# Ascend-Research/HeadPoseEstimation-WHENet

Hardware: NVIDIA H100
Metric: head-crops/sec @224x224 bf16 (higher is better)
Workload: dtype bf16

## Files before the change

headposeestimation-whenet_b200/csrc/kernels_simt.cuh:

```cuda
#pragma once
#include <cuda_bf16.h>
#include <cuda_fp16.h>
#include <cuda_runtime.h>
#include <stdint.h>

namespace whenet {

template <typename T> struct Store;
template <> struct Store<float> {
    static constexpr int VEC = 4;
    __device__ static __forceinline__ float ld(const float* p) { return *p; }
    __device__ static __forceinline__ void st(float* p, float v) { *p = v; }
    __device__ static __forceinline__ float rnd(float v) { return v; }
};
template <> struct Store<__nv_bfloat16> {
    static constexpr int VEC = 8;
    __device__ static __forceinline__ float ld(const __nv_bfloat16* p) { return __bfloat162float(*p); }
    __device__ static __forceinline__ void st(__nv_bfloat16* p, float v) { *p = __float2bfloat16_rn(v); }
    __device__ static __forceinline__ float rnd(float v) { return __bfloat162float(__float2bfloat16_rn(v)); }
};
template <> struct Store<__half> {
    static constexpr int VEC = 8;
    __device__ static __forceinline__ float ld(const __half* p) { return __half2float(*p); }
    __device__ static __forceinline__ void st(__half* p, float v) { *p = __float2half_rn(v); }
    __device__ static __forceinline__ float rnd(float v) { return __half2float(__float2half_rn(v)); }
};

__device__ __forceinline__ void ld4(const float* p, float (&v)[4]) {
    float4 t = *reinterpret_cast<const float4*>(p);
    v[0] = t.x; v[1] = t.y; v[2] = t.z; v[3] = t.w;
}
__device__ __forceinline__ void ld4(const __nv_bfloat16* p, float (&v)[4]) {
    uint2 t = *reinterpret_cast<const uint2*>(p);
    __nv_bfloat162 a = *reinterpret_cast<__nv_bfloat162*>(&t.x), b = *reinterpret_cast<__nv_bfloat162*>(&t.y);
    float2 fa = __bfloat1622float2(a), fb = __bfloat1622float2(b);
    v[0] = fa.x; v[1] = fa.y; v[2] = fb.x; v[3] = fb.y;
}
__device__ __forceinline__ void ld4(const __half* p, float (&v)[4]) {
    uint2 t = *reinterpret_cast<const uint2*>(p);
    __half2 a = *reinterpret_cast<__half2*>(&t.x), b = *reinterpret_cast<__half2*>(&t.y);
    float2 fa = __half22float2(a), fb = __half22float2(b);
    v[0] = fa.x; v[1] = fa.y; v[2] = fb.x; v[3] = fb.y;
}
__device__ __forceinline__ void st4(float* p, const float (&v)[4]) {
    *reinterpret_cast<float4*>(p) = make_float4(v[0], v[1], v[2], v[3]);
}
__device__ __forceinline__ void st4(__nv_bfloat16* p, const float (&v)[4]) {
    __nv_bfloat162 a = __floats2bfloat162_rn(v[0], v[1]), b = __floats2bfloat162_rn(v[2], v[3]);
    uint2 t; t.x = *reinterpret_cast<uint32_t*>(&a); t.y = *reinterpret_cast<uint32_t*>(&b);
    *reinterpret_cast<uint2*>(p) = t;
}
__device__ __forceinline__ void st4(__half* p, const float (&v)[4]) {
    __half2 a = __floats2half2_rn(v[0], v[1]), b = __floats2half2_rn(v[2], v[3]);
    uint2 t; t.x = *reinterpret_cast<uint32_t*>(&a); t.y = *reinterpret_cast<uint32_t*>(&b);
    *reinterpret_cast<uint2*>(p) = t;
}

template <typename T> __device__ __forceinline__ void ld8(const T* p, float (&v)[8]) {
    float a[4], b[4];
    ld4(p, a); ld4(p + 4, b);
#pragma unroll
    for (int i = 0; i < 4; ++i) { v[i] = a[i]; v[4 + i] = b[i]; }
}
template <> __device__ __forceinline__ void ld8<__nv_bfloat16>(const __nv_bfloat16* p, float (&v)[8]) {
    uint4 t = *reinterpret_cast<const uint4*>(p);
    const __nv_bfloat162* h = reinterpret_cast<const __nv_bfloat162*>(&t);
#pragma unroll
    for (int i = 0; i < 4; ++i) { float2 f = __bfloat1622float2(h[i]); v[2 * i] = f.x; v[2 * i + 1] = f.y; }
}
template <> __device__ __forceinline__ void ld8<__half>(const __half* p, float (&v)[8]) {
    uint4 t = *reinterpret_cast<const uint4*>(p);
    const __half2* h = reinterpret_cast<const __half2*>(&t);
#pragma unroll
    for (int i = 0; i < 4; ++i) { float2 f = __half22float2(h[i]); v[2 * i] = f.x; v[2 * i + 1] = f.y; }
}
template <typename T> __device__ __forceinline__ void st8(T* p, const float (&v)[8]) {
    float a[4] = {v[0], v[1], v[2], v[3]}, b[4] = {v[4], v[5], v[6], v[7]};
    st4(p, a); st4(p + 4, b);
}
template <> __device__ __forceinline__ void st8<__nv_bfloat16>(__nv_bfloat16* p, const float (&v)[8]) {
    uint4 t; __nv_bfloat162* h = reinterpret_cast<__nv_bfloat162*>(&t);
#pragma unroll
    for (int i = 0; i < 4; ++i) h[i] = __floats2bfloat162_rn(v[2 * i], v[2 * i + 1]);
    *reinterpret_cast<uint4*>(p) = t;
}
template <> __device__ __forceinline__ void st8<__half>(__half* p, const float (&v)[8]) {
    uint4 t; __half2* h = reinterpret_cast<__half2*>(&t);
#pragma unroll
    for (int i = 0; i < 4; ++i) h[i] = __floats2half2_rn(v[2 * i], v[2 * i + 1]);
    *reinterpret_cast<uint4*>(p) = t;
}

__device__ __forceinline__ float swish_f(float x) { return x / (1.0f + expf(-x)); }
__device__ __forceinline__ float sigmoid_f(float x) { return 1.0f / (1.0f + expf(-x)); }
__device__ __forceinline__ float swish_fast(float x) {
    const float h = 0.5f * x;
    float t;
    asm("tanh.approx.f32 %0, %1;" : "=f"(t) : "f"(h));
    return fmaf(h, t, h);
}

__device__ __forceinline__ float swish_from_half(float h) {
    float t;
    asm("tanh.approx.f32 %0, %1;" : "=f"(t) : "f"(h));
    return fmaf(h, t, h);
}

template <typename T, bool IN_U8>
__global__ void __launch_bounds__(256) stem_kernel(const void* __restrict__ in_, T* __restrict__ out,
                                                   const float* __restrict__ w,
                                                   const float* __restrict__ bias,
                                                   const float* __restrict__ lut,
                                                   int n_img) {
    __shared__ float s_w[27 * 32];
    __shared__ float s_lut[3 * 256];
    for (int i = threadIdx.x; i < 27 * 32; i += 256) s_w[i] = w[i];
    if (IN_U8)
        for (int i = threadIdx.x; i < 768; i += 256) s_lut[i] = lut[i];
    __syncthreads();
    const long long total = (long long)n_img * 112 * 112 * 4;
    long long gid = (long long)blockIdx.x * 256 + threadIdx.x;
    if (gid >= total) return;
    const int cg = (int)(gid & 3);
    long long pix = gid >> 2;
    const int ox = (int)(pix % 112); pix /= 112;
    const int oy = (int)(pix % 112);
    const int n = (int)(pix / 112);
    float acc[8];
#pragma unroll
    for (int i = 0; i < 8; ++i) acc[i] = bias[cg * 8 + i];
#pragma unroll
    for (int ky = 0; ky < 3; ++ky) {
        const int iy = 2 * oy + ky;
        if (iy >= 224) continue;
#pragma unroll
        for (int kx = 0; kx < 3; ++kx) {
            const int ix = 2 * ox + kx;
            if (ix >= 224) continue;
            const long long base = (((long long)n * 224 + iy) * 224 + ix) * 3;
#pragma unroll
            for (int ci = 0; ci < 3; ++ci) {
                float x;
                if (IN_U8) x = s_lut[ci * 256 + reinterpret_cast<const uint8_t*>(in_)[base + ci]];
                else x = reinterpret_cast<const float*>(in_)[base + ci];
                const float* wr = &s_w[((ky * 3 + kx) * 3 + ci) * 32 + cg * 8];
#pragma unroll
                for (int i = 0; i < 8; ++i) acc[i] = fmaf(x, wr[i], acc[i]);
            }
        }
    }
#pragma unroll
    for (int i = 0; i < 8; ++i) acc[i] = swish_f(acc[i]);
    st8(out + (gid >> 2) * 32 + cg * 8, acc);
}

struct StemParams { float w[27 * 32]; float b[32]; };

template <typename T, bool IN_U8, bool FAST>
__global__ void __launch_bounds__(224) stem_tile_kernel(const void* __restrict__ in_, T* __restrict__ out,
                                                        const __grid_constant__ StemParams sp,
                                                        const float* __restrict__ lut) {
    constexpr int ROWF = 225 * 3 + 1;
    __shared__ float s_in[5 * ROWF];
    __shared__ float s_lut[768];
    const int tid = threadIdx.x;
    const int n = blockIdx.y, oy0 = blockIdx.x * 2;
    if (IN_U8) {
        for (int i = tid; i < 768; i += 224) s_lut[i] = lut[i];
        __syncthreads();
    }
    if (IN_U8) {
        const uint8_t* src = reinterpret_cast<const uint8_t*>(in_) + (long long)n * 224 * 224 * 3;
        for (int v = tid; v < 5 * 42; v += 224) {
            const int r = v / 42, q = v - r * 42;
            const int iy = 2 * oy0 + r;
            float* dst = &s_in[r * ROWF + q * 16];
            if (iy < 224) {
                const uint4 raw = *reinterpret_cast<const uint4*>(src + (long long)iy * 672 + q * 16);
                const uint8_t* b = reinterpret_cast<const uint8_t*>(&raw);
#pragma unroll
                for (int j = 0; j < 16; ++j) dst[j] = s_lut[((q * 16 + j) % 3) * 256 + b[j]];
            } else {
#pragma unroll
                for (int j = 0; j < 16; ++j) dst[j] = 0.f;
            }
        }
    } else {
        const float* src = reinterpret_cast<const float*>(in_) + (long long)n * 224 * 224 * 3;
        for (int v = tid; v < 5 * 168; v += 224) {
            const int r = v / 168, q = v - r * 168;
            const int iy = 2 * oy0 + r;
            float4 x = make_float4(0.f, 0.f, 0.f, 0.f);
            if (iy < 224) x = *reinterpret_cast<const float4*>(src + (long long)iy * 672 + q * 4);
            float* dst = &s_in[r * ROWF + q * 4];
            dst[0] = x.x; dst[1] = x.y; dst[2] = x.z; dst[3] = x.w;
        }
    }
    if (tid < 15) s_in[(tid / 3) * ROWF + 672 + tid % 3] = 0.f;
    __syncthreads();
    const int oyl = tid / 112, ox = tid - oyl * 112;
    float2 acc2[16];
#pragma unroll
    for (int c = 0; c < 16; ++c) acc2[c] = make_float2(sp.b[2 * c], sp.b[2 * c + 1]);
#pragma unroll
    for (int ky = 0; ky < 3; ++ky) {
        const float* row = &s_in[(2 * oyl + ky) * ROWF + 6 * ox];
#pragma unroll
        for (int t = 0; t < 9; ++t) {
            const float x = row[t];
            const float2 xx = make_float2(x, x);
#pragma unroll
            for (int c = 0; c < 16; ++c) {
                const float2 w2 = make_float2(sp.w[(ky * 9 + t) * 32 + 2 * c], sp.w[(ky * 9 + t) * 32 + 2 * c + 1]);
                acc2[c].x = fmaf(xx.x, w2.x, acc2[c].x);
                acc2[c].y = fmaf(xx.y, w2.y, acc2[c].y);
            }
        }
    }
    float acc[32];
#pragma unroll
    for (int c = 0; c < 16; ++c) { acc[2 * c] = acc2[c].x; acc[2 * c + 1] = acc2[c].y; }
    T* dst = out + (((long long)n * 112 + oy0 + oyl) * 112 + ox) * 32;
#pragma unroll
    for (int g = 0; g < 4; ++g) {
        float o[8];
#pragma unroll
        for (int j = 0; j < 8; ++j) o[j] = FAST ? swish_fast(acc[g * 8 + j]) : swish_f(acc[g * 8 + j]);
        st8<T>(dst + g * 8, o);
    }
}

template <typename T, bool SWISH, bool GATE, bool RESID>
__global__ void __launch_bounds__(256) pw_conv_kernel(const T* __restrict__ A, const float* __restrict__ W,
                                                      const float* __restrict__ bias, const float* __restrict__ gate,
                                                      const T* __restrict__ resid, T* __restrict__ out,
                                                      long long M, int K, int N, int hw) {
    constexpr int BM = 64, BN = 64, BK = 16;
    __shared__ float As[BK][BM + 4];
    __shared__ float Bs[BK][BN];
    const int tid = threadIdx.x;
    const int tx = tid & 15, ty = tid >> 4;
    const long long m0 = (long long)blockIdx.x * BM;
    const int n0 = blockIdx.y * BN;
    float acc[4][4];
#pragma unroll
    for (int i = 0; i < 4; ++i)
#pragma unroll
        for (int j = 0; j < 4; ++j) acc[i][j] = 0.f;

    const int a_row = tid >> 2, a_k = (tid & 3) * 4;
    const int b_k = tid >> 4, b_n = (tid & 15) * 4;
    const long long a_m = m0 + a_row;
    const bool a_ok = a_m < M;
    const float* gate_row = GATE ? gate + (a_ok ? (a_m / hw) : 0) * K : nullptr;

    for (int k0 = 0; k0 < K; k0 += BK) {
        float av[4] = {0.f, 0.f, 0.f, 0.f};
        if (a_ok && k0 + a_k < K) {
            ld4(A + a_m * K + k0 + a_k, av);
            if (GATE) {
                float g[4]; ld4(gate_row + k0 + a_k, g);
#pragma unroll
                for (int i = 0; i < 4; ++i) av[i] *= g[i];
            }
        }
#pragma unroll
        for (int i = 0; i < 4; ++i) As[a_k + i][a_row] = av[i];
        float4 bv = make_float4(0.f, 0.f, 0.f, 0.f);
        if (k0 + b_k < K && n0 + b_n < N) bv = *reinterpret_cast<const float4*>(W + (long long)(k0 + b_k) * N + n0 + b_n);
        *reinterpret_cast<float4*>(&Bs[b_k][b_n]) = bv;
        __syncthreads();
#pragma unroll
        for (int k = 0; k < BK; ++k) {
            float4 a4 = *reinterpret_cast<const float4*>(&As[k][ty * 4]);
            float4 b4 = *reinterpret_cast<const float4*>(&Bs[k][tx * 4]);
            const float a[4] = {a4.x, a4.y, a4.z, a4.w}, b[4] = {b4.x, b4.y, b4.z, b4.w};
#pragma unroll
            for (int i = 0; i < 4; ++i)
#pragma unroll
                for (int j = 0; j < 4; ++j) acc[i][j] = fmaf(a[i], b[j], acc[i][j]);
        }
        __syncthreads();
    }
    const int n = n0 + tx * 4;
    if (n >= N) return;
    float bb[4]; ld4(bias + n, bb);
#pragma unroll
    for (int i = 0; i < 4; ++i) {
        const long long m = m0 + ty * 4 + i;
        if (m >= M) break;
        float v[4];
#pragma unroll
        for (int j = 0; j < 4; ++j) {
            float x = acc[i][j] + bb[j];
            v[j] = SWISH ? swish_f(x) : x;
        }
        if (RESID) {
            float r[4]; ld4(resid + m * N + n, r);
#pragma unroll
            for (int j = 0; j < 4; ++j) v[j] += r[j];
        }
        st4(out + m * N + n, v);
    }
}

template <typename T, int KS, int S>
__global__ void __launch_bounds__(256) dw_conv_kernel(const T* __restrict__ in, const float* __restrict__ w,
                                                      const float* __restrict__ bias, T* __restrict__ out,
                                                      float* __restrict__ partial,
                                                      int Hin, int Ho, int C, int pad, int rows) {
    extern __shared__ float s_red[];
    const int cv = threadIdx.x, py = threadIdx.y, PY = blockDim.y;
    const int c0 = cv * 8;
    const int n = blockIdx.y, tile = blockIdx.x;
    const int r0 = tile * rows;
    const int r1 = min(Ho, r0 + rows);
    const int npix = (r1 - r0) * Ho;
    const T* in_n = in + (long long)n * Hin * Hin * C;
    T* out_n = out + (long long)n * Ho * Ho * C;
    float bb[8];
#pragma unroll
    for (int i = 0; i < 8; ++i) bb[i] = bias[c0 + i];
    float sum[8];
#pragma unroll
    for (int i = 0; i < 8; ++i) sum[i] = 0.f;
    for (int p = py; p < npix; p += PY) {
        const int oy = r0 + p / Ho, ox = p % Ho;
        float acc[8];
#pragma unroll
        for (int i = 0; i < 8; ++i) acc[i] = bb[i];
#pragma unroll
        for (int ky = 0; ky < KS; ++ky) {
            const int iy = oy * S + ky - pad;
            if (iy < 0 || iy >= Hin) continue;
#pragma unroll
            for (int kx = 0; kx < KS; ++kx) {
                const int ix = ox * S + kx - pad;
                if (ix < 0 || ix >= Hin) continue;
                float x[8], ww[8];
                ld8(in_n + ((long long)iy * Hin + ix) * C + c0, x);
                ld8(w + (ky * KS + kx) * C + c0, ww);
#pragma unroll
                for (int i = 0; i < 8; ++i) acc[i] = fmaf(x[i], ww[i], acc[i]);
            }
        }
#pragma unroll
        for (int i = 0; i < 8; ++i) { acc[i] = swish_f(acc[i]); }
        st8(out_n + ((long long)oy * Ho + ox) * C + c0, acc);
#pragma unroll
        for (int i = 0; i < 8; ++i) sum[i] += Store<T>::rnd(acc[i]);
    }
#pragma unroll
    for (int i = 0; i < 8; ++i) s_red[py * C + c0 + i] = sum[i];
    __syncthreads();
    if (py == 0) {
        float tot[8];
#pragma unroll
        for (int i = 0; i < 8; ++i) tot[i] = 0.f;
        for (int y = 0; y < PY; ++y)
#pragma unroll
            for (int i = 0; i < 8; ++i) tot[i] += s_red[y * C + c0 + i];
        float* dst = partial + ((long long)n * gridDim.x + tile) * C + c0;
#pragma unroll
        for (int i = 0; i < 8; ++i) dst[i] = tot[i];
    }
}


template <typename T, int KS, int S, int R, bool FAST>
__global__ void __launch_bounds__(256) dw_strip_kernel(const T* __restrict__ in, const float* __restrict__ w,
                                                       const float* __restrict__ bias, T* __restrict__ out,
                                                       float* __restrict__ partial,
                                                       int Hin, int Ho, int C, int pad, int rows) {
    extern __shared__ float s_red[];
    constexpr int NCOL = (R - 1) * S + KS;
    const int cv = threadIdx.x, py = threadIdx.y, PY = blockDim.y;
    const int c0 = cv * 8;
    const int n = blockIdx.y, tile = blockIdx.x;
    const int r0 = tile * rows;
    const int r1 = min(Ho, r0 + rows);
    const int spr = (Ho + R - 1) / R;
    const int nstrips = (r1 - r0) * spr;
// ... 409 lines not shown
```

headposeestimation-whenet_b200/csrc/whenet_api.cu:

```cuda
#include <cuda_bf16.h>
#include <cuda_fp16.h>
#include <cuda_runtime.h>

#include <algorithm>
#include <atomic>
#include <cmath>
#include <cstdarg>
#include <cstdio>
#include <cstdlib>
#include <cstring>
#include <map>
#include <string>
#include <thread>
#include <type_traits>
#include <vector>

#include "../../include/whenet_b200.h"
#include "api_error.h"
#include "kernels_simt.cuh"
#include "kernels_tc.cuh"
#include "kernels_fused.cuh"
#include "kernels_crop.cuh"
#include "kernels_overlay.cuh"
#include "kernels_k2.cuh"
// ... 356 lines not shown
int make_tmap_kd_e(CUtensorMap* tm, const void* base, int n, int H, int C, int cc, int pw) {
    auto fn = tmap_encode_fn();
    if (!fn) return fail(WHENET_ECUDA, "cuTensorMapEncodeTiled is not available from this driver");
    const cuuint64_t dims[4] = {(cuuint64_t)C, (cuuint64_t)H, (cuuint64_t)H, (cuuint64_t)n};
    const cuuint64_t strides[3] = {(cuuint64_t)C * 2, (cuuint64_t)H * C * 2, (cuuint64_t)H * H * C * 2};
    const cuuint32_t box[4] = {(cuuint32_t)cc, (cuuint32_t)pw, (cuuint32_t)pw, 1};
    const cuuint32_t estr[4] = {1, 1, 1, 1};
    const CUresult r = fn(tm, CU_TENSOR_MAP_DATA_TYPE_FLOAT16, 4, const_cast<void*>(base), dims, strides, box, estr, CU_TENSOR_MAP_INTERLEAVE_NONE,
                          CU_TENSOR_MAP_SWIZZLE_NONE, CU_TENSOR_MAP_L2_PROMOTION_L2_128B, CU_TENSOR_MAP_FLOAT_OOB_FILL_NONE);
    if (r != CUDA_SUCCESS) return fail(WHENET_ECUDA, "cuTensorMapEncodeTiled(KD tile %dx%dx%dx%d, box %dx%dx%d) failed: %d", n, H, H, C, pw, pw, cc, (int)r);
    return 0;
}
int make_tmap_k1x_in(CUtensorMap* tm, const void* base, int n, int H, int C, int iw, int row_bytes) {
    auto fn = tmap_encode_fn();
    if (!fn) return fail(WHENET_ECUDA, "cuTensorMapEncodeTiled is not available from this driver");
    const cuuint64_t dims[4] = {(cuuint64_t)C, (cuuint64_t)H, (cuuint64_t)H, (cuuint64_t)n};
    const cuuint64_t strides[3] = {(cuuint64_t)C * 2, (cuuint64_t)H * C * 2, (cuuint64_t)H * H * C * 2};
    const cuuint32_t box[4] = {(cuuint32_t)row_bytes / 2, (cuuint32_t)iw, (cuuint32_t)iw, 1};
    const cuuint32_t estr[4] = {1, 1, 1, 1};
    const CUresult r = fn(tm, CU_TENSOR_MAP_DATA_TYPE_BFLOAT16, 4, const_cast<void*>(base), dims, strides, box, estr, CU_TENSOR_MAP_INTERLEAVE_NONE,
                          row_bytes == 64 ? CU_TENSOR_MAP_SWIZZLE_64B : CU_TENSOR_MAP_SWIZZLE_128B, CU_TENSOR_MAP_L2_PROMOTION_L2_128B,
                          CU_TENSOR_MAP_FLOAT_OOB_FILL_NONE);
    if (r != CUDA_SUCCESS) return fail(WHENET_ECUDA, "cuTensorMapEncodeTiled(K1X input %dx%dx%dx%d, box %dx%d) failed: %d", n, H, H, C, iw, iw, (int)r);
    return 0;
}
int make_tmap_kd_w(CUtensorMap* tm, const void* base, int kk, int C, int cc) {
    auto fn = tmap_encode_fn();
    if (!fn) return fail(WHENET_ECUDA, "cuTensorMapEncodeTiled is not available from this driver");
    const cuuint64_t dims[2] = {(cuuint64_t)C, (cuuint64_t)kk};
    const cuuint64_t strides[1] = {(cuuint64_t)C * 2};
    const cuuint32_t box[2] = {(cuuint32_t)cc, (cuuint32_t)kk};
    const cuuint32_t estr[2] = {1, 1};
    const CUresult r = fn(tm, CU_TENSOR_MAP_DATA_TYPE_FLOAT16, 2, const_cast<void*>(base), dims, strides, box, estr, CU_TENSOR_MAP_INTERLEAVE_NONE,
                          CU_TENSOR_MAP_SWIZZLE_NONE, CU_TENSOR_MAP_L2_PROMOTION_L2_128B, CU_TENSOR_MAP_FLOAT_OOB_FILL_NONE);
    if (r != CUDA_SUCCESS) return fail(WHENET_ECUDA, "cuTensorMapEncodeTiled(KD weights %dx%d, box %d) failed: %d", kk, C, cc, (int)r);
    return 0;
}

template <typename T>
int launch_pw(whenet_ctx* c, const char* name, const T* A, const float* W, const void* Wt16, const float* bias,
              const float* gate, const T* resid, T* out, long long M, int K, int N, int hw, bool swish, bool out_half = false) {
    const double bytes = (double)M * (K + N + (resid ? N : 0)) * sizeof(T);
    const double flops = 2.0 * (double)M * K * N;
    Scope sc(c, name, bytes, flops);
    if constexpr (sizeof(T) == 2) {
        const bool want_k2 = c->pw_variant == 3 || (c->pw_variant == 4 && (gate == nullptr || hw <= 196));
        if (c->use_tc && Wt16 && want_k2 && !out_half) {
            whenet::tc::K2Params kp{};
            size_t smem = 0;
            if (whenet::tc::plan_k2(M, K, N, hw, gate != nullptr, c->precision == WHENET_PRECISION_BF16, &kp, &smem) &&
                (c->pw_variant == 3 || kp.tiles >= 2 * c->sm_count)) {
                if (c->tmaps2.size() > 1024) c->tmaps2.clear();
                const TmapKey ka{K, (int)M, (const void*)A}, kw{-N, K, Wt16};
                auto ia = c->tmaps2.find(ka);
                if (ia == c->tmaps2.end()) {
                    CUtensorMap tm;
                    int rc = make_tmap_w(&tm, A, (int)M, K, whenet::tc::BM, c->precision == WHENET_PRECISION_BF16);
                    if (rc) return rc;
                    ia = c->tmaps2.emplace(ka, tm).first;
                }
                auto iw = c->tmaps2.find(kw);
                if (iw == c->tmaps2.end()) {
                    CUtensorMap tm;
                    int rc = make_tmap_w(&tm, Wt16, N, K, kp.n_tile, c->precision == WHENET_PRECISION_BF16);
                    if (rc) return rc;
                    iw = c->tmaps2.emplace(kw, tm).first;
                }
                kp.tmA = ia->second; kp.tmW = iw->second;
                kp.bias = bias; kp.gate = gate; kp.resid = resid; kp.out = out; kp.tflag = c->d_tflag;
                int rc = whenet::tc::launch_k2<T>(c->stream, kp, smem, swish, gate != nullptr, resid != nullptr, c->sm_count);
                if (rc == 0) { CK(cudaGetLastError()); return 0; }
                if (rc < 0) return fail(WHENET_ECUDA, "K2 launch failed for %s (rc=%d)", name, rc);
            }
        }
        if (c->use_tc && Wt16 && gate && hw >= 784 && c->pw3 && !out_half && !swish) {
            int rc = whenet::tc::launch_pw_tc3<T>(c->stream, A, Wt16, bias, gate, resid, out, M, K, N, hw);
            if (rc == 0) { CK(cudaGetLastError()); return 0; }
            if (rc < 0) return fail(WHENET_ECUDA, "pw_tc3 launch failed for %s (rc=%d)", name, rc);
        }
        if (c->use_tc && Wt16) {
            int rc = whenet::tc::launch_pw_tc2<T>(c->stream, A, Wt16, bias, gate, resid, out, M, K, N, hw, swish, c->pw_stage_cap, c->pw_smem_kb, c->pw_min_ctas, out_half);
            if (rc == 0) { CK(cudaGetLastError()); return 0; }
            if (rc < 0) return fail(WHENET_ECUDA, "tensor-core 1x1 launch failed for %s (rc=%d)", name, rc);
        }
    }
    if constexpr (sizeof(T) == 4) {
        if (c->use_tc && Wt16 && c->split_lo_bytes) {
            int rc = whenet::tc::launch_pw_tc32(c->stream, A, Wt16, (const char*)Wt16 + c->split_lo_bytes, bias, gate, resid, out, M, K, N, hw, swish);
            if (rc == 0) { CK(cudaGetLastError()); return 0; }
            if (rc < 0) return fail(WHENET_ECUDA, "split-bf16 tensor-core 1x1 launch failed for %s (rc=%d)", name, rc);
        }
    }
    if (out_half) return fail(WHENET_EINVAL, "fp16-output 1x1 conv needs the tensor-core kernel (%s)", name);
    dim3 grid((unsigned)((M + 63) / 64), (unsigned)((N + 63) / 64));
#define PW(SW, GA, RE) whenet::pw_conv_kernel<T, SW, GA, RE><<<grid, 256, 0, c->stream>>>(A, W, bias, gate, resid, out, M, K, N, hw)
    if (swish && !gate && !resid) PW(true, false, false);
    else if (!swish && gate && !resid) PW(false, true, false);
    else if (!swish && gate && resid) PW(false, true, true);
    else if (!swish && !gate && !resid) PW(false, false, false);
    else if (!swish && !gate && resid) PW(false, false, true);
    else return fail(WHENET_EINVAL, "unsupported 1x1 epilogue combination");
#undef PW
    CK(cudaGetLastError());
    return 0;
}

template <typename T>
int launch_dw(whenet_ctx* c, const char* name, const BlockCfg& b, const BlockW& w, const T* in, T* out, int nb, int* tiles_out) {
    const int rows = b.hout >= 28 ? 8 : b.hout;
    const int tiles = (b.hout + rows - 1) / rows;
    *tiles_out = tiles;
    const int cv = b.cexp / 8;
    const int py = std::max(1, 256 / cv);
    dim3 grid(tiles, nb), block(cv, py);
    const size_t smem = (size_t)py * b.cexp * sizeof(float);
    const double bytes = (double)nb * ((double)b.hin * b.hin + (double)b.hout * b.hout) * b.cexp * sizeof(T);
    const double flops = 2.0 * nb * (double)b.hout * b.hout * b.k * b.k * b.cexp;
    Scope sc(c, name, bytes, flops);
#define DW(KS, S) whenet::dw_conv_kernel<T, KS, S><<<grid, block, smem, c->stream>>>(in, w.w_dw, w.b_dw, out, c->d_partial, b.hin, b.hout, b.cexp, b.pad, rows)
#define DWS(KS, S, R) whenet::dw_strip_kernel<T, KS, S, R, (sizeof(T) == 2)><<<grid, block, smem, c->stream>>>(in, w.w_dw, w.b_dw, out, c->d_partial, b.hin, b.hout, b.cexp, b.pad, rows)
    if (c->dw_variant == 0) {
        if (b.k == 3 && b.s == 1) DW(3, 1);
        else if (b.k == 3 && b.s == 2) DW(3, 2);
        else if (b.k == 5 && b.s == 1) DW(5, 1);
        else if (b.k == 5 && b.s == 2) DW(5, 2);
        else return fail(WHENET_EINVAL, "unsupported depthwise config");
    } else {
        if (b.k == 3 && b.s == 1) { if (b.hout % 4 == 0) DWS(3, 1, 4); else DWS(3, 1, 7); }
        else if (b.k == 3 && b.s == 2) { if (b.hout % 4 == 0) DWS(3, 2, 4); else DWS(3, 2, 7); }
        else if (b.k == 5 && b.s == 1) { if (b.hout % 4 == 0) DWS(5, 1, 4); else DWS(5, 1, 7); }
        else if (b.k == 5 && b.s == 2) { if (b.hout % 4 == 0) DWS(5, 2, 4); else DWS(5, 2, 7); }
        else return fail(WHENET_EINVAL, "unsupported depthwise config");
    }
#undef DWS
#undef DW
    CK(cudaGetLastError());
    return 0;
}

template <typename T, bool IN_U8>
int forward_chunk(whenet_ctx* c, const void* d_in, int nb, float* d_angles, float* d_logits, bool taps, int off) {
    char nm[48];
    const bool plain_dw = taps && c->taps_mode == 1;
    T* cur = (T*)c->bufA;
    T* oth = (T*)c->bufB;
    T* E = (T*)c->bufE;
    T* D = (T*)c->bufD;
    const bool stem_half = std::is_same<T, __nv_bfloat16>::value && c->use_fused && c->use_tc && c->dw1_kd && c->stem_variant != 0 && !c->blocks.empty() &&
                           !c->blocks[0].has_expand && c->blocks[0].cexp == 32 && c->blocks[0].k == 3 && c->blocks[0].s == 1 && c->blocks[0].hin % 14 == 0;
    {
        Scope sc(c, "stem", (double)nb * (kImgElems * (IN_U8 ? 1.0 : 4.0) + 112.0 * 112 * 32 * sizeof(T)),
                 2.0 * nb * 112.0 * 112 * 27 * 32);
        if (stem_half) {
            whenet::stem_tile_kernel<__half, IN_U8, true><<<dim3(56, nb), 224, 0, c->stream>>>(d_in, reinterpret_cast<__half*>(cur), c->stem_params, c->lut);
        } else if (c->stem_variant == 0) {
            const long long total = (long long)nb * 112 * 112 * 4;
            whenet::stem_kernel<T, IN_U8><<<(unsigned)((total + 255) / 256), 256, 0, c->stream>>>(d_in, cur, c->w_stem, c->b_stem, c->lut, nb);
        } else {
            whenet::stem_tile_kernel<T, IN_U8, (sizeof(T) == 2)><<<dim3(56, nb), 224, 0, c->stream>>>(d_in, cur, c->stem_params, c->lut);
        }
        CK(cudaGetLastError());
    }
    if (taps) {
        int rc = stem_half ? add_tap<__half>(c, "stem", reinterpret_cast<const __half*>(cur), (size_t)112 * 112 * 32, off, nb)
                           : add_tap<T>(c, "stem", cur, (size_t)112 * 112 * 32, off, nb);
        if (rc) return rc;
    }
    for (size_t i = 0; i < c->blocks.size(); ++i) {
        const BlockCfg& b = c->blocks[i];
        const BlockW& w = c->bw[i];
        const T* dw_in = cur;
        int tiles = 0;
        bool did_k1 = false;
        bool se_in_k1 = false;
        bool d_gated = false;
        const bool use_kd = std::is_same<T, __nv_bfloat16>::value && c->use_fused && c->use_tc && c->kd_from > 0 && b.idx >= c->kd_from &&
                            b.has_expand && whenet::fused::dwse_chunk(b.k, b.s, b.hin, b.cexp) > 0;
        if constexpr (sizeof(T) == 2) {
            if (i == 0 && stem_half) {
              if constexpr (std::is_same<T, __nv_bfloat16>::value) {
                whenet::fused::DwSeParams p{};
                if (c->tmaps.size() > 512) c->tmaps.clear();
                const TmapKey ke{100 + b.idx, nb, (const void*)cur}, kw{200 + b.idx, 0, (const void*)w.w_dw16};
                auto ie = c->tmaps.find(ke);
                if (ie == c->tmaps.end()) {
                    CUtensorMap tm;
                    int rc = make_tmap_kd_e(&tm, cur, nb, b.hin, b.cexp, 32, 16);
                    if (rc) return rc;
                    ie = c->tmaps.emplace(ke, tm).first;
                }
                auto iw = c->tmaps.find(kw);
                if (iw == c->tmaps.end()) {
                    CUtensorMap tm;
                    int rc = make_tmap_kd_w(&tm, w.w_dw16, 9, b.cexp, 32);
                    if (rc) return rc;
                    iw = c->tmaps.emplace(kw, tm).first;
                }
                p.tmE = ie->second; p.tmW = iw->second;
                p.b_dw = w.b_dw_h; p.tflag = c->d_tflag; p.out = D; p.partial = c->d_partial;
                p.C = b.cexp; p.pad = b.pad; p.Cse = b.cse; p.inv_hw = 1.0f / (float)(b.hout * b.hout);
                int split = 1;
                {
                    const int n_tiles = (b.hin / 14) * (b.hin / 14);
                    while (split < n_tiles && (long long)nb * split < c->k1_split_ctas) ++split;
                }
                snprintf(nm, sizeof nm, "b%02d.dw", b.idx);
                Scope sc(c, nm, (double)nb * 2.0 * b.hin * b.hin * b.cexp * sizeof(T), 2.0 * nb * (double)b.hout * b.hout * b.k * b.k * b.cexp);
                int rc = whenet::fused::launch_dwse_spatial<T>(c->stream, p, b.hin, nb, split);
                if (rc != 0) return fail(WHENET_ECUDA, "KD (block 1) launch failed (rc=%d)", rc);
                CK(cudaGetLastError());
                tiles = (b.hin / 14) * (b.hin / 14);
                did_k1 = true;
              }
            } else if (i == 0 && !did_k1 && c->use_fused && c->dw1_fused && c->dw1.valid) {
                whenet::fused::K1Params p = c->dw1.p;
                p.in = cur; p.wt_aug = nullptr; p.w_dw = w.w_dw_h; p.b_dw = w.b_dw_h; p.out = D; p.partial = c->d_partial; p.tflag = c->d_tflag;
                p.w_se1t = w.w_se1t; p.b_se1 = w.b_se1; p.w_se2 = w.w_se2; p.b_se2 = w.b_se2; p.gate = c->d_gate; p.Cse = b.cse;
                se_in_k1 = c->se_fused != 0;
                p.se_counter = se_in_k1 ? c->d_se_counter : nullptr;
                snprintf(nm, sizeof nm, "b%02d.dw", b.idx);
                Scope sc(c, nm, (double)nb * 2.0 * b.hin * b.hin * b.cexp * sizeof(T), 2.0 * nb * (double)b.hout * b.hout * b.k * b.k * b.cexp);
                int rc = whenet::fused::launch_dw_only<T>(c->stream, p, c->dw1.smem, nb);
                if (rc != 0) return fail(WHENET_ECUDA, "depthwise-only K1 launch failed (rc=%d)", rc);
                CK(cudaGetLastError());
                tiles = p.tiles_x * p.tiles_y;
                did_k1 = true;
            } else if (use_kd) {
              if constexpr (std::is_same<T, __nv_bfloat16>::value) {
                const int cc = whenet::fused::dwse_chunk(b.k, b.s, b.hin, b.cexp);
                int split = 1;
                while (split < b.cexp / cc && (long long)nb * split < c->k1_split_ctas) ++split;
                int rc = 0;
                if (split > 1) {
                    snprintf(nm, sizeof nm, "b%02d.expand", b.idx);
                    rc = launch_pw<T>(c, nm, cur, w.w_exp, w.wt_exp, w.b_exp, nullptr, nullptr, E,
                                      (long long)nb * b.hin * b.hin, b.cin, b.cexp, b.hin * b.hin, true, true);
                    if (rc) return rc;
                }
                whenet::fused::DwSeParams p{};
                {
                    const int pw = (b.hout - 1) * b.s + b.k;
                    if (c->tmaps.size() > 512) c->tmaps.clear();
                    const TmapKey kw{200 + b.idx, 0, (const void*)w.w_dw16};
                    auto iw = c->tmaps.find(kw);
                    if (iw == c->tmaps.end()) {
                        CUtensorMap tm;
                        if ((rc = make_tmap_kd_w(&tm, w.w_dw16, b.k * b.k, b.cexp, cc))) return rc;
                        iw = c->tmaps.emplace(kw, tm).first;
                    }
                    p.tmW = iw->second;
                    if (split > 1) {
                        const TmapKey ke{100 + b.idx, nb, (const void*)E};
                        auto ie = c->tmaps.find(ke);
                        if (ie == c->tmaps.end()) {
                            CUtensorMap tm;
                            if ((rc = make_tmap_kd_e(&tm, E, nb, b.hin, b.cexp, cc, pw))) return rc;
                            ie = c->tmaps.emplace(ke, tm).first;
                        }
                        p.tmE = ie->second;
                    } else {
                        const TmapKey kx{300 + b.idx, nb, (const void*)cur}, kwx{400 + b.idx, 0, (const void*)w.wt_exp};
                        auto ix = c->tmaps.find(kx);
                        if (ix == c->tmaps.end()) {
                            CUtensorMap tm;
                            if ((rc = make_tmap_w(&tm, cur, nb * b.hin * b.hin, b.cin, (b.hin * b.hin + 7) / 8 * 8, true))) return rc;
                            ix = c->tmaps.emplace(kx, tm).first;
                        }
                        auto iwx = c->tmaps.find(kwx);
                        if (iwx == c->tmaps.end()) {
                            CUtensorMap tm;
                            if ((rc = make_tmap_w(&tm, w.wt_exp, b.cexp, b.cin, cc, true))) return rc;
                            iwx = c->tmaps.emplace(kwx, tm).first;
                        }
                        p.tmX = ix->second; p.tmWx = iwx->second;
                        p.b_exp = w.b_exp;
                    }
                }
                p.b_dw = w.b_dw_h; p.tflag = c->d_tflag;
                p.out = D; p.partial = c->d_partial;
                p.w_se1t = w.w_se1t; p.b_se1 = w.b_se1; p.w_se2 = w.w_se2; p.b_se2 = w.b_se2; p.gate = c->d_gate; p.Cse = b.cse;
                p.inv_hw = 1.0f / (float)(b.hout * b.hout);
                p.C = b.cexp; p.pad = b.pad;
                if (split == 1 && c->se_tail && c->kd_tail) {
                    p.se_tail = 1;
                    se_in_k1 = true;
                    if (c->se_scale_out && !plain_dw) { p.scale_out = 1; d_gated = true; }
                }
                snprintf(nm, sizeof nm, "b%02d.kd", b.idx);
                if (split == 1) {
                    Scope sc(c, nm, (double)nb * ((double)b.hin * b.hin * b.cin + (double)b.hout * b.hout * b.cexp) * sizeof(T),
                             2.0 * nb * ((double)b.hin * b.hin * b.cin * b.cexp + (double)b.hout * b.hout * b.k * b.k * b.cexp));
                    rc = whenet::fused::launch_dwse_x<T>(c->stream, p, b.k, b.s, b.hin, b.cin, nb);
                    if (rc != 0) return fail(WHENET_ECUDA, "KD (on-chip expand) launch failed for block %d (rc=%d)", b.idx, rc);
                    CK(cudaGetLastError());
                } else {
                    Scope sc(c, nm, (double)nb * ((double)b.hin * b.hin + (double)b.hout * b.hout) * b.cexp * sizeof(T),
                             2.0 * nb * (double)b.hout * b.hout * b.k * b.k * b.cexp);
                    rc = whenet::fused::launch_dwse<T>(c->stream, p, b.k, b.s, b.hin, nb, split);
                    if (rc != 0) return fail(WHENET_ECUDA, "KD launch failed for block %d (rc=%d)", b.idx, rc);
                    CK(cudaGetLastError());
                }
                tiles = 1;
                did_k1 = true;
              }
            } else if (c->use_fused && c->k1[i].valid && b.idx <= c->fused_max_block) {
                whenet::fused::K1Params p = c->k1[i].p;
                p.in = cur; p.wt_aug = w.wt_exp_aug; p.w_dw = w.w_dw_h; p.w_dw16 = w.w_dw16; p.b_dw = w.b_dw_h; p.out = D; p.partial = c->d_partial; p.tflag = c->d_tflag;
                p.w_se1t = w.w_se1t; p.b_se1 = w.b_se1; p.w_se2 = w.w_se2; p.b_se2 = w.b_se2; p.gate = c->d_gate; p.Cse = b.cse;
                se_in_k1 = c->se_fused && p.NB == 1;
                p.se_counter = se_in_k1 ? c->d_se_counter : nullptr;
                {
                    const long long ctas = (long long)p.tiles_x * p.tiles_y * ((nb + p.NB - 1) / p.NB);
                    int split = 1;
                    while (split < p.n_chunks && ctas * split < c->k1_split_ctas) ++split;
// ... 1382 lines not shown
```

Measured before the change: 84300.

## Rewrite stem conv as persistent tiled kernel with cp.async prefetch and staged stores

The stem tile kernel becomes persistent: a grid sized to occupancy loops over 8-row tiles. The next tile's raw input is prefetched with cp.async into shared memory while the current tile computes. Input is rearranged into stride-2 column planes so each thread computes 4 output pixels with float4 loads. Weights are held in shared memory, and outputs are staged through a swizzled shared buffer so global writes coalesce. This targets the stem's memory latency and uncoalesced stores, at the cost of more dynamic shared memory, extra syncs and a per-launch occupancy query on the host.

Result: faster. 87150, median of 6 (+3.4%).

```diff
diff --git a/headposeestimation-whenet_b200/csrc/kernels_simt.cuh b/headposeestimation-whenet_b200/csrc/kernels_simt.cuh
--- a/headposeestimation-whenet_b200/csrc/kernels_simt.cuh
+++ b/headposeestimation-whenet_b200/csrc/kernels_simt.cuh
@@ -3,6 +3,8 @@
 #include <cuda_fp16.h>
 #include <cuda_runtime.h>
 #include <stdint.h>
+
+#include <algorithm>
 
 namespace whenet {
 
@@ -156,78 +158,160 @@
 
 struct StemParams { float w[27 * 32]; float b[32]; };
 
+constexpr int kStemRows = 8;
+constexpr int kStemTilesPerCrop = 112 / kStemRows;
+constexpr int kStemThreads = kStemRows * 28;
+constexpr int kStemPlane = 112;
+constexpr int kStemRowF = 9 * kStemPlane + 8;
+constexpr int kStemInRows = 2 * kStemRows + 1;
+
+template <typename T, bool IN_U8>
+struct StemSmem {
+    static constexpr size_t PLANES = (size_t)kStemInRows * kStemRowF * 4;
+    static constexpr size_t RAW_ROW = 672 * (IN_U8 ? 1 : 4);
+    static constexpr size_t STAGE = (size_t)kStemRows * 112 * 16 * sizeof(T);
+    static constexpr size_t RAW = (size_t)kStemInRows * RAW_ROW;
+    static constexpr size_t UNION = STAGE > RAW ? STAGE : RAW;
+    static constexpr size_t LUT = PLANES + UNION, W = LUT + (IN_U8 ? 768 * 4 : 0);
+    static constexpr size_t BYTES = W + 27 * 32 * 4;
+};
+
+template <int HALF, typename T, bool FAST>
+__device__ __forceinline__ void stem_half(const float* s_in, const float* s_w, uint4* stage, T* out_run, int q, int tid,
+                                          const StemParams& sp) {
+    float acc[4][16];
+#pragma unroll
+    for (int c = 0; c < 16; ++c)
+#pragma unroll
+        for (int p = 0; p < 4; ++p) acc[p][c] = sp.b[HALF * 16 + c];
+    const int oyl = q / 28;
+    const float* x0 = s_in + 2 * oyl * kStemRowF + 4 * (q - oyl * 28);
+#pragma unroll
+    for (int ky = 0; ky < 3; ++ky)
+#pragma unroll
+        for (int t = 0; t < 9; ++t) {
+            const float4 x = *reinterpret_cast<const float4*>(x0 + ky * kStemRowF + t * kStemPlane);
+            const float xs[4] = {x.x, x.y, x.z, x.w};
+            float ws[16];
+#pragma unroll
+            for (int c4 = 0; c4 < 4; ++c4) {
+                const float4 w4 = *reinterpret_cast<const float4*>(s_w + (ky * 9 + t) * 32 + HALF * 16 + 4 * c4);
+                ws[4 * c4] = w4.x; ws[4 * c4 + 1] = w4.y; ws[4 * c4 + 2] = w4.z; ws[4 * c4 + 3] = w4.w;
+            }
+#pragma unroll
+            for (int c = 0; c < 16; ++c)
+#pragma unroll
+                for (int p = 0; p < 4; ++p) acc[p][c] = fmaf(xs[p], ws[c], acc[p][c]);
+        }
+    if (HALF == 1) __syncthreads();
+    constexpr int CPH = (int)sizeof(T);
+    constexpr int SH = CPH == 2 ? 3 : 4;
+    constexpr int VPC = 16 / (int)sizeof(T);
+#pragma unroll
+    for (int p = 0; p < 4; ++p)
+#pragma unroll
+        for (int j = 0; j < CPH; ++j) {
+            const int k = (q * 4 + p) * CPH + j;
+            float o[VPC];
+#pragma unroll
+            for (int e = 0; e < VPC; ++e) o[e] = FAST ? swish_fast(acc[p][j * VPC + e]) : swish_f(acc[p][j * VPC + e]);
+            T* dst = reinterpret_cast<T*>(stage + (k ^ ((k >> SH) & 7)));
+            if constexpr (sizeof(T) == 2) st8<T>(dst, o);
+            else st4(dst, o);
+        }
+    __syncthreads();
+    uint4* g = reinterpret_cast<uint4*>(out_run + HALF * 16);
+#pragma unroll
+    for (int k = tid; k < kStemRows * 112 * CPH; k += kStemThreads)
+        g[(k / CPH) * 2 * CPH + k % CPH] = stage[k ^ ((k >> SH) & 7)];
+}
+
+template <bool IN_U8>
+__device__ __forceinline__ void stem_fetch(const void* in_, char* raw, int tile, int tid) {
+    constexpr int ROW = 672 * (IN_U8 ? 1 : 4), CPR = ROW / 16;
+    const int n = tile / kStemTilesPerCrop, oy0 = (tile - n * kStemTilesPerCrop) * kStemRows;
+    const int rows = min(kStemInRows, 224 - 2 * oy0);
+    const char* src = reinterpret_cast<const char*>(in_) + ((long long)n * 224 + 2 * oy0) * ROW;
+    for (int i = tid; i < rows * CPR; i += kStemThreads) {
+        const uint32_t dst = (uint32_t)__cvta_generic_to_shared(raw + i * 16);
+        asm volatile("cp.async.cg.shared.global [%0], [%1], 16;" ::"r"(dst), "l"(src + (long long)i * 16) : "memory");
+    }
+    asm volatile("cp.async.commit_group;" ::: "memory");
+}
+
 template <typename T, bool IN_U8, bool FAST>
-__global__ void __launch_bounds__(224) stem_tile_kernel(const void* __restrict__ in_, T* __restrict__ out,
-                                                        const __grid_constant__ StemParams sp,
-                                                        const float* __restrict__ lut) {
-    constexpr int ROWF = 225 * 3 + 1;
-    __shared__ float s_in[5 * ROWF];
-    __shared__ float s_lut[768];
+__global__ void __launch_bounds__(kStemThreads, 2) stem_tile_kernel(const void* __restrict__ in_, T* __restrict__ out,
+                                                                    const __grid_constant__ StemParams sp,
+                                                                    const float* __restrict__ lut, int n_img) {
+    using S = StemSmem<T, IN_U8>;
+    extern __shared__ float4 stem_smem_v[];
+    char* base = reinterpret_cast<char*>(stem_smem_v);
+    float* s_in = reinterpret_cast<float*>(base);
+    char* s_raw = base + S::PLANES;
+    uint4* stage0 = reinterpret_cast<uint4*>(base + S::PLANES);
+    float* s_lut = reinterpret_cast<float*>(base + S::LUT);
+    float* s_w = reinterpret_cast<float*>(base + S::W);
     const int tid = threadIdx.x;
-    const int n = blockIdx.y, oy0 = blockIdx.x * 2;
-    if (IN_U8) {
-        for (int i = tid; i < 768; i += 224) s_lut[i] = lut[i];
+    const int tiles = n_img * kStemTilesPerCrop;
+    int tile = blockIdx.x;
+    if (tile < tiles) stem_fetch<IN_U8>(in_, s_raw, tile, tid);
+    for (int i = tid; i < 27 * 32; i += kStemThreads) s_w[i] = sp.w[i];
+    if (IN_U8)
+        for (int i = tid; i < 768; i += kStemThreads) s_lut[i] = lut[i];
+    for (; tile < tiles; tile += gridDim.x) {
+        const int n = tile / kStemTilesPerCrop, oy0 = (tile - n * kStemTilesPerCrop) * kStemRows;
+        asm volatile("cp.async.wait_group 0;" ::: "memory");
         __syncthreads();
-    }
-    if (IN_U8) {
-        const uint8_t* src = reinterpret_cast<const uint8_t*>(in_) + (long long)n * 224 * 224 * 3;
-        for (int v = tid; v < 5 * 42; v += 224) {
-            const int r = v / 42, q = v - r * 42;
-            const int iy = 2 * oy0 + r;
-            float* dst = &s_in[r * ROWF + q * 16];
-            if (iy < 224) {
-                const uint4 raw = *reinterpret_cast<const uint4*>(src + (long long)iy * 672 + q * 16);
-                const uint8_t* b = reinterpret_cast<const uint8_t*>(&raw);
-#pragma unroll
-                for (int j = 0; j < 16; ++j) dst[j] = s_lut[((q * 16 + j) % 3) * 256 + b[j]];
-            } else {
-#pragma unroll
-                for (int j = 0; j < 16; ++j) dst[j] = 0.f;
-            }
-        }
-    } else {
-        const float* src = reinterpret_cast<const float*>(in_) + (long long)n * 224 * 224 * 3;
-        for (int v = tid; v < 5 * 168; v += 224) {
-            const int r = v / 168, q = v - r * 168;
-            const int iy = 2 * oy0 + r;
-            float4 x = make_float4(0.f, 0.f, 0.f, 0.f);
-            if (iy < 224) x = *reinterpret_cast<const float4*>(src + (long long)iy * 672 + q * 4);
-            float* dst = &s_in[r * ROWF + q * 4];
-            dst[0] = x.x; dst[1] = x.y; dst[2] = x.z; dst[3] = x.w;
-        }
-    }
-    if (tid < 15) s_in[(tid / 3) * ROWF + 672 + tid % 3] = 0.f;
-    __syncthreads();
-    const int oyl = tid / 112, ox = tid - oyl * 112;
-    float2 acc2[16];
-#pragma unroll
-    for (int c = 0; c < 16; ++c) acc2[c] = make_float2(sp.b[2 * c], sp.b[2 * c + 1]);
-#pragma unroll
-    for (int ky = 0; ky < 3; ++ky) {
-        const float* row = &s_in[(2 * oyl + ky) * ROWF + 6 * ox];
-#pragma unroll
-        for (int t = 0; t < 9; ++t) {
-            const float x = row[t];
-            const float2 xx = make_float2(x, x);
-#pragma unroll
-            for (int c = 0; c < 16; ++c) {
-                const float2 w2 = make_float2(sp.w[(ky * 9 + t) * 32 + 2 * c], sp.w[(ky * 9 + t) * 32 + 2 * c + 1]);
-                acc2[c].x = fmaf(xx.x, w2.x, acc2[c].x);
-                acc2[c].y = fmaf(xx.y, w2.y, acc2[c].y);
-            }
-        }
-    }
-    float acc[32];
-#pragma unroll
-    for (int c = 0; c < 16; ++c) { acc[2 * c] = acc2[c].x; acc[2 * c + 1] = acc2[c].y; }
-    T* dst = out + (((long long)n * 112 + oy0 + oyl) * 112 + ox) * 32;
-#pragma unroll
-    for (int g = 0; g < 4; ++g) {
-        float o[8];
-#pragma unroll
-        for (int j = 0; j < 8; ++j) o[j] = FAST ? swish_fast(acc[g * 8 + j]) : swish_f(acc[g * 8 + j]);
-        st8<T>(dst + g * 8, o);
-    }
+        for (int i = tid; i < kStemInRows * 112; i += kStemThreads) {
+            const int r = i / 112, m = i - r * 112;
+            float v[6] = {0.f, 0.f, 0.f, 0.f, 0.f, 0.f};
+            if (2 * oy0 + r < 224) {
+                const char* src = s_raw + r * S::RAW_ROW;
+#pragma unroll
+                for (int k = 0; k < 3; ++k) {
+                    if (IN_U8) {
+                        const uint16_t u = reinterpret_cast<const uint16_t*>(src + 6 * m)[k];
+                        v[2 * k] = s_lut[((2 * k) % 3) * 256 + (u & 0xff)];
+                        v[2 * k + 1] = s_lut[((2 * k + 1) % 3) * 256 + (u >> 8)];
+                    } else {
+                        const float2 f = reinterpret_cast<const float2*>(src + 24 * m)[k];
+                        v[2 * k] = f.x; v[2 * k + 1] = f.y;
+                    }
+                }
+            }
+            float* row = s_in + r * kStemRowF;
+#pragma unroll
+            for (int ci = 0; ci < 3; ++ci) {
+                row[ci * kStemPlane + m] = v[ci];
+                row[(3 + ci) * kStemPlane + m] = v[3 + ci];
+                if (m > 0) row[(6 + ci) * kStemPlane + m - 1] = v[ci];
+                else row[(6 + ci) * kStemPlane + 111] = 0.f;
+            }
+        }
+        __syncthreads();
+        T* out_run = out + ((long long)n * 112 + oy0) * 112 * 32;
+        stem_half<0, T, FAST>(s_in, s_w, stage0, out_run, tid, tid, sp);
+        __syncthreads();
+        if (tile + (int)gridDim.x < tiles) stem_fetch<IN_U8>(in_, s_raw, tile + gridDim.x, tid);
+        stem_half<1, T, FAST>(s_in, s_w, reinterpret_cast<uint4*>(base), out_run, tid, tid, sp);
+    }
+    asm volatile("cp.async.wait_group 0;" ::: "memory");
+}
+
+template <typename T, bool IN_U8, bool FAST>
+cudaError_t launch_stem_tile(cudaStream_t stream, const void* in, T* out, const StemParams& sp, const float* lut, int n) {
+    auto kfn = stem_tile_kernel<T, IN_U8, FAST>;
+    constexpr size_t smem = StemSmem<T, IN_U8>::BYTES;
+    cudaError_t e = cudaFuncSetAttribute(kfn, cudaFuncAttributeMaxDynamicSharedMemorySize, (int)smem);
+    int dev = 0, sms = 0, per_sm = 0;
+    if (e == cudaSuccess) e = cudaGetDevice(&dev);
+    if (e == cudaSuccess) e = cudaDeviceGetAttribute(&sms, cudaDevAttrMultiProcessorCount, dev);
+    if (e == cudaSuccess) e = cudaOccupancyMaxActiveBlocksPerMultiprocessor(&per_sm, kfn, kStemThreads, smem);
+    if (e != cudaSuccess) return e;
+    if (per_sm < 1) return cudaErrorInvalidConfiguration;
+    const long long tiles = (long long)n * kStemTilesPerCrop;
+    kfn<<<(unsigned)std::min(tiles, (long long)per_sm * sms), kStemThreads, smem, stream>>>(in, out, sp, lut, n);
+    return cudaGetLastError();
 }
 
 template <typename T, bool SWISH, bool GATE, bool RESID>
diff --git a/headposeestimation-whenet_b200/csrc/whenet_api.cu b/headposeestimation-whenet_b200/csrc/whenet_api.cu
--- a/headposeestimation-whenet_b200/csrc/whenet_api.cu
+++ b/headposeestimation-whenet_b200/csrc/whenet_api.cu
@@ -532,14 +532,14 @@
         Scope sc(c, "stem", (double)nb * (kImgElems * (IN_U8 ? 1.0 : 4.0) + 112.0 * 112 * 32 * sizeof(T)),
                  2.0 * nb * 112.0 * 112 * 27 * 32);
         if (stem_half) {
-            whenet::stem_tile_kernel<__half, IN_U8, true><<<dim3(56, nb), 224, 0, c->stream>>>(d_in, reinterpret_cast<__half*>(cur), c->stem_params, c->lut);
+            CK((whenet::launch_stem_tile<__half, IN_U8, true>(c->stream, d_in, reinterpret_cast<__half*>(cur), c->stem_params, c->lut, nb)));
         } else if (c->stem_variant == 0) {
             const long long total = (long long)nb * 112 * 112 * 4;
             whenet::stem_kernel<T, IN_U8><<<(unsigned)((total + 255) / 256), 256, 0, c->stream>>>(d_in, cur, c->w_stem, c->b_stem, c->lut, nb);
+            CK(cudaGetLastError());
         } else {
-            whenet::stem_tile_kernel<T, IN_U8, (sizeof(T) == 2)><<<dim3(56, nb), 224, 0, c->stream>>>(d_in, cur, c->stem_params, c->lut);
-        }
-        CK(cudaGetLastError());
+            CK((whenet::launch_stem_tile<T, IN_U8, (sizeof(T) == 2)>(c->stream, d_in, cur, c->stem_params, c->lut, nb)));
+        }
     }
     if (taps) {
         int rc = stem_half ? add_tap<__half>(c, "stem", reinterpret_cast<const __half*>(cur), (size_t)112 * 112 * 32, off, nb)
```
